# SpectacularAI/HybVIO

Measured on AMD Instinct MI355X. Metric: VIO frames/sec at 752x480 stereo, 200 KLT features; pyramid+KLT HBM GB/s, higher is better.
Workload: dtype u8/int16 pixels, int32/int64 sums, f32 solve (tracker); f64 (EKF); 1 GPU; C3: 752x480 stereo, 200 pts -- the whole frame chained on one stream per sequence: 2 pyramid builds, temporal LK from predicted positions, 2-point rotation RANSAC on its output, stereo LK, GFTT key points every 2nd frame (HIP tracker), then the HIP EKF from the device mean: 20 track visits (triangulation + prepareVisualUpdate + chi2 gate; track lengths 5 + Geometric(0.2) <= 21 stereo poses = 20 .~; sequences_per_gpu=4096, engines_per_gpu=4, parallelism=replicas x1 (no collective)

## Files before the change

### hybvio_amd/csrc/ekf.hip

```cpp
#include <functional>
#include <limits.h>
#include <math.h>

#include <utility>

#include <stdlib.h>

#include "ekf_device.hpp"

#pragma clang fp contract(fast)

namespace hv {

namespace {


}
__device__ long long g_phase_stamp[16];
namespace {
#ifdef HV_EKF_PHASE_STAMPS
#define PHASE_STAMP(i) do { if (blockIdx.x == 0 && threadIdx.x == 0) g_phase_stamp[i] = (long long)__builtin_readcyclecounter(); } while (0)
#else
#define PHASE_STAMP(i) do { } while (0)
#endif
// ... 496 lines not shown
        }
        __syncthreads();
        for (int w = t; w < ns * 12; w += 256) {
            const int sl = w / 12, tt = w - 12 * sl;
            double *const sh = shs + sl * SHW;
            if (sh[X_LIVE] == 0.0) continue;
            double *const F = Fs + sl * INER * INER;
            const double *const sA = sh, *const sT34 = sh + 88;
            const int i = tt / 4, j = tt - 4 * i;
            double s_ = 0; for (int k = 0; k < 4; k++) s_ += sT34[3 * k + i] * sA[4 * j + k];
            F_(VEL + i, ORI + j) = s_;
        }
        __syncthreads();
        for (int w = t; w < ns * 32; w += 256) {
            const int sl = w >> 5, tt = w & 31;
            double *const sh = shs + sl * SHW;
            if (sh[X_LIVE] == 0.0) continue;
            double *const F = Fs + sl * INER * INER, *const Lm = Ls + sl * INER * QD;
            if (tt < 9) {
                const int i = tt / 3, g = tt - 3 * i;
                double s_ = 0; for (int k = 0; k < 4; k++) s_ += F_(VEL + i, ORI + k) * L_(ORI + k, Q_GYRO + g);
                L_(VEL + i, Q_GYRO + g) = s_;
                F_(VEL + i, BGA + g) = -s_;
            } else if (tt >= 16 && tt < 28) {
                const int e = tt - 16, i = e / 3, g = e - 3 * i;
                F_(ORI + i, BGA + g) = -L_(ORI + i, Q_GYRO + g);
            }
        }
        if (s0 == 0) PHASE_STAMP(6);
        int last_live = -1;
        bool q_set = false;
        auto set_q = [&](const double *sh_q) {
            if (a.baa > 0.0 && t < 9) { const int i = t % 3, j = t / 3; Qs[(Q_BAA_DRIFT + j) * QD + Q_BAA_DRIFT + i] = (i == j) ? sh_q[X_VBAA] : 0.0; }
            if (a.bga > 0.0 && t >= 16 && t < 25) { const int e = t - 16, i = e % 3, j = e / 3; Qs[(Q_BGA_DRIFT + j) * QD + Q_BGA_DRIFT + i] = (i == j) ? sh_q[X_VBGA] : 0.0; }
        };
        for (int sl = 0; sl < ns; sl++) {
            double *const sh = shs + sl * SHW;
            __syncthreads();
            if (sh[X_LIVE] == 0.0) continue;
            last_live = sl;
            const double *const F = Fs + sl * INER * INER, *const Lm = Ls + sl * INER * QD;
            if (!q_set) { set_q(sh); __syncthreads(); }
            q_set = false;
            if (s0 == 0 && sl == 1) PHASE_STAMP(7);
            const int ti = wave & 1, tj = wave >> 1;
            const int mi = ti ? INER - 16 : 16, nj = tj ? INER - 16 : 16;
            const double4v fp = mfma_tile<5>(F + 16 * ti, 1, INER, mi, P00 + 16 * tj * INER, 1, INER, nj, INER);
            const double4v ph = mfma_tile<5>(F + 16 * ti, 1, INER, mi, Phi + 16 * tj * INER, 1, INER, nj, INER);
            double4v lq = {0.0, 0.0, 0.0, 0.0};
            if (wave < 2) lq = mfma_tile<3>(Lm + 16 * wave, 1, INER, wave ? INER - 16 : 16, Qs, 1, QD, QD, QD);
#pragma unroll
            for (int q = 0; q < 4; q++) {
                const int r = kq + 4 * q;
                if (r < mi && cl < nj) { FP[(16 * tj + cl) * INER + 16 * ti + r] = fp[q]; PhiN[(16 * tj + cl) * INER + 16 * ti + r] = ph[q]; }
                if (wave < 2 && r < (wave ? INER - 16 : 16) && cl < QD) LQ[cl * INER + 16 * wave + r] = lq[q];
            }
            if (s0 == 0 && sl == 1) PHASE_STAMP(8);
            __syncthreads();
            if (s0 == 0 && sl == 1) PHASE_STAMP(9);
            {
                int nx = sl + 1;
                while (nx < ns && shs[nx * SHW + X_LIVE] == 0.0) nx++;
                if (nx < ns) { set_q(shs + nx * SHW); q_set = true; }
            }
            const double4v p1 = mfma_tile<5>(FP + 16 * ti, 1, INER, mi, F + 16 * tj, INER, 1, nj, INER);
            const double4v p2 = mfma_tile<3>(LQ + 16 * ti, 1, INER, mi, Lm + 16 * tj, INER, 1, nj, QD);
#pragma unroll
            for (int q = 0; q < 4; q++) {
                const int r = kq + 4 * q;
                if (r < mi && cl < nj) P00[(16 * tj + cl) * INER + 16 * ti + r] = p1[q] + p2[q];
            }
            for (int e = t; e < INER * INER; e += 256) Phi[e] = PhiN[e];
            if (s0 == 0 && sl == 1) PHASE_STAMP(10);
        }
        __syncthreads();
        if (s0 == 0) PHASE_STAMP(11);
        if (last_live >= 0)
            for (int i = t; i < INER * INER; i += 256) a.dydx[(size_t)b * INER * INER + i] = Fs[last_live * INER * INER + i];
        __syncthreads();
    }
    for (int i = t; i < INER * INER; i += 256) P[(size_t)(i / INER) * n + (i % INER)] = P00[i];
    for (int i = t; i < QD * QD; i += 256) Q[i] = Qs[i];
    if (t < INER) m[t] = ms[t];
    PHASE_STAMP(14);
    {
        double f0[5], f1[5];
#pragma unroll
        for (int sx = 0; sx < 5; sx++) {
            const int k = 4 * sx + kq;
            f0[sx] = Phi[k * INER + cl];
            f1[sx] = Phi[k * INER + min(16 + cl, INER - 1)];
        }
        for (int base = 0; base < 2 * tiles; base += 4 * NIT) {
#pragma unroll
            for (int u = 0; u < NIT; u++) {
                const int it = base + wave + 4 * u;
                if (it < 2 * tiles) {
                    if (base > 0) {
#pragma unroll
                        for (int sx = 0; sx < 5; sx++) slab[u][sx] = *slab_ptr(it, sx);
                    }
                    double4v a0 = {0.0, 0.0, 0.0, 0.0}, a1 = a0;
                    const bool p10 = it < tiles;
#pragma unroll
                    for (int sx = 0; sx < 5; sx++) {
                        const double x0 = p10 ? f0[sx] : slab[u][sx], y0 = p10 ? slab[u][sx] : f0[sx];
                        const double x1 = p10 ? f1[sx] : slab[u][sx], y1 = p10 ? slab[u][sx] : f1[sx];
                        a0 = __builtin_amdgcn_mfma_f64_16x16x4f64(x0, y0, a0, 0, 0, 0);
                        a1 = __builtin_amdgcn_mfma_f64_16x16x4f64(x1, y1, a1, 0, 0, 0);
                    }
#pragma unroll
                    for (int q = 0; q < 4; q++) {
                        const int rr = kq + 4 * q;
                        if (p10) {
                            const int i = INER + 16 * it + cl;
                            if (i < n) {
                                P[(size_t)rr * n + i] = a0[q];
                                if (16 + rr < INER) P[(size_t)(16 + rr) * n + i] = a1[q];
                            }
                        } else {
                            const int c = INER + 16 * (it - tiles) + rr;
                            if (c < n) {
                                P[(size_t)c * n + cl] = a0[q];
                                if (16 + cl < INER) P[(size_t)c * n + 16 + cl] = a1[q];
                            }
                        }
                    }
                }
            }
        }
    }
    __syncthreads();
    PHASE_STAMP(15);
}

struct UpdateArgs {
    int n, nr, l, R, Rs;
    int mode;
    int generic;
    int normalize_all, use_lds, map_dim;
    double *m, *P;
    const double *H, *v;
    const double *rdiag;
    double rd0, noise_scale;
    double rd1;
    double *ws;
    double *chi2; int *status;
    const unsigned char *active;
    const int *require_inlier;
    int *success_counter;
    int spec, n_tracks, max_successful;
    int *cursor;
    const int *gate_in;
    const int *nr_rec;
    int *cursor_out;
    int *pub;
    int pass_id;
    int *err;
    const int *acol;
    int na_max, ncam;
    size_t h_stride;
    int v_stride;
    int half, nr_full;
    double *dm_out; const double *dm_in;
    int *gate_rw;
    int half_auto; int *sel_io;
    int *epoch;
    int batch;
    const int *rec_count, *rec_list;
};

__device__ __forceinline__ void spec_publish(const UpdateArgs &a, int rec, int code)
{
    __hip_atomic_store(a.pub + rec, a.pass_id * 4 + code, __ATOMIC_RELEASE, __HIP_MEMORY_SCOPE_AGENT);
}
__device__ __forceinline__ int spec_wait(const UpdateArgs &a, int rec)
{
    for (int spin = 0; spin < (1 << 20); ++spin) {
        const int v = __hip_atomic_load(a.pub + rec, __ATOMIC_ACQUIRE, __HIP_MEMORY_SCOPE_AGENT);
        if ((v >> 2) == a.pass_id) return v & 3;
        __builtin_amdgcn_s_sleep(8);
    }
    if (a.err) atomicOr(a.err, 1);
    return -1;
}
__device__ __forceinline__ void spec_close(const UpdateArgs &a, int b, int c0, bool pass_ran)
{
    bool any = false;
    for (int jj = c0; jj < a.n_tracks - 1 && !any; ++jj) any = spec_wait(a, jj * (int)gridDim.x + b) == 2;
    if (!any) a.cursor_out[b] = pass_ran ? a.n_tracks : c0;
}

constexpr int UPD_THREADS = 512;

template <int MODE, int TI, bool AUTO = false>
__device__ __forceinline__ void ekf_update_body(const UpdateArgs &a, const int b_in )
{
    const int b = __builtin_amdgcn_readfirstlane(b_in);
    constexpr bool USE_LDS = MODE >= 1;
    extern __shared__ __attribute__((aligned(16))) double smem[];
    int e = b;
    int sel = -1;
    if (a.spec == 1) {
        const int j = blockIdx.y;
        if (j < a.cursor[b] || a.success_counter[b] >= a.max_successful) return;
        e = j * (int)gridDim.x + b;
    } else if (AUTO && a.spec == 2 && a.half == 2) {
        sel = a.sel_io[b];
        if (sel < 0) return;
        e = sel * (int)gridDim.x + b;
        if (a.gate_in[e] != 0) {
            if (threadIdx.x == 0) a.cursor[b] = sel + 1;
            return;
        }
    } else if (a.spec == 2) {
        const int c0 = a.cursor[b];
        if (AUTO && threadIdx.x == 0) a.sel_io[b] = -1;
        if (c0 >= a.n_tracks || a.success_counter[b] >= a.max_successful) return;
        for (int j = c0; j < a.n_tracks && sel < 0; ++j) {
            const int ee = j * (int)gridDim.x + b;
            if (a.active[ee] && a.gate_in[ee] == 0) sel = j;
        }
        if (sel < 0) {
            __syncthreads();
            if (threadIdx.x == 0) a.cursor[b] = a.n_tracks;
            return;
        }
        e = sel * (int)gridDim.x + b;
    }
    int c0_spec = 0;
    if (a.spec == 3) {
        const int j = blockIdx.y;
        c0_spec = a.cursor[b];
        e = j * (int)gridDim.x + b;
        const bool pass_runs = c0_spec < a.n_tracks && a.success_counter[b] < a.max_successful;
        if (!pass_runs || j < c0_spec || !a.active[e]) {
            if (threadIdx.x == 0) {
                spec_publish(a, e, 1);
                if (j == a.n_tracks - 1) spec_close(a, b, c0_spec, pass_runs);
            }
            return;
        }
    }
    const int t = threadIdx.x, lane = t & 63;
    const unsigned char act_v = a.active ? a.active[e] : (unsigned char)1;
    const int req_v = a.require_inlier ? a.require_inlier[b] : 0;
    const int nr_rec_v0 = a.nr_rec ? a.nr_rec[e] : a.nr_full;
    int shape_pin = nr_rec_v0;
    asm volatile("" : "+v"(shape_pin));
    const int nr_rec_v = shape_pin;
    if (!act_v) return;
    if (req_v != 0) return;
#ifdef HV_DEBUG_SKIP_UPDATE
    if (a.mode == 1 && a.spec == 0) { if (a.success_counter && t == 0) a.success_counter[b] += 1; return; }
#endif
    const int wave = __builtin_amdgcn_readfirstlane(t >> 6);
    constexpr int nwaves = UPD_THREADS / 64;
    const int n = a.n, l = a.l;
    int nr = a.nr, R = a.Rs, Rfull = a.R;
    int roff = 0, ld = a.nr;
    int half = a.half;
    if (a.nr_rec || a.half) {
        int nr_full = __builtin_amdgcn_readfirstlane(nr_rec_v);
        if (nr_full < 1 || nr_full > a.v_stride) return;
        nr = nr_full; ld = nr_full;
        if constexpr (AUTO) {
            if (nr_full <= 48) {
                if (half == 2) return;
                half = 0;
            }
            if (half == 1 && t == 0) a.sel_io[b] = sel;
        }
        if (half) {
            if (MODE != 2) return;
            const int h1 = 2 * ((nr_full + 3) >> 2);
            roff = half == 2 ? h1 : 0;
            nr = half == 2 ? nr_full - h1 : h1;
        }
        if (nr < 1 || nr > a.nr) return;
        Rfull = nr + n + 1; R = Rfull;
        if (USE_LDS) while ((R & 31) != 15 && (R & 31) != 17) R++;
    }
    double *m = a.m + (size_t)b * n, *P = a.P + (size_t)b * n * n;
    const double *H = a.H + (size_t)e * a.h_stride;
    const double rd = a.rdiag ? a.rdiag[b] : a.rd0;
    double *T = USE_LDS ? smem : a.ws + (size_t)b * a.Rs * a.nr;
    double *W = USE_LDS ? smem + (((size_t)R * nr + 1) & ~(size_t)1) : smem;
    double *col = W + 256;
    double *red = col + 544;
    int *s_stop = reinterpret_cast<int *>(red + nwaves);
    double *Hs = red + nwaves + 2;
    constexpr int nrp = 16 * (TI > 0 ? TI : 1);
    const bool gate_only = a.mode == 0;
    const int rv = nr, ry = nr + 1;
    const bool two_r = MODE == 2 && a.mode == 3;
    int Rlim = (gate_only || two_r) ? nr + 1 : Rfull;

    PHASE_STAMP(0);
    const int kq = lane >> 4, cl = lane & 15;
    constexpr int NBK = 10, NBH = 5;
    double pres0[NBK][4], pres1[NBH][4];
    const int tiles_j = (n + 15) >> 4, lb = (l + 15) >> 4;
    const int hs = (tiles_j + 1) >> 1;
    const int J1 = 8 + (wave & 1), kb0_1 = (wave & 2) ? hs : 0, kb1_1 = (wave & 2) ? tiles_j : hs;
    const bool have0 = MODE == 2 && wave < tiles_j, have1 = MODE == 2 && wave < 4 && J1 < tiles_j;
    unsigned kbmask = 0xFFFFFFFFu;
    if constexpr (MODE == 2) {
        auto fetch_blk = [&](auto &pv, int bi, int J, int kb, int kend) {
            if (kb < kend && (kb < lb || !gate_only)) {
                const int jc = min(J * 16 + cl, n - 1);
#pragma unroll
                for (int sx = 0; sx < 4; sx++)
                    pv[bi][sx] = *reinterpret_cast<const double *>(reinterpret_cast<const char *>(P) + (unsigned)(min(kb * 16 + 4 * sx + kq, n - 1) * n + jc) * 8u);
            }
        };
        constexpr int HREG = (48 * 160 + UPD_THREADS - 1) / UPD_THREADS, DEPTH = 4;
        if (a.acol) {
            int *mask = reinterpret_cast<int *>(col);
            const int na = 7 * (ld / (2 * a.ncam)) + 1;
            const int *acol = a.acol + (size_t)e * a.na_max;
            const int total = na * nr;
            const unsigned inv_nr = (unsigned)((0x100000000ull + (unsigned)nr - 1) / (unsigned)nr);
            constexpr int HC = 8;
            double hv[HC]; int hc[HC];
            auto request = [&](int base) {
#pragma unroll
                for (int u = 0; u < HC; u++) {
                    const int i = base + t + u * UPD_THREADS, uc = (int)__umulhi((unsigned)i, inv_nr), r = i - uc * nr;
                    const bool live = i < total;
                    hc[u] = live ? acol[uc] : -1;
                    hv[u] = live ? *reinterpret_cast<const double *>(reinterpret_cast<const char *>(H) + (unsigned)(uc * ld + roff + r) * 8u) : 0.0;
                }
            };
            auto scatter = [&](int base) {
#pragma unroll
                for (int u = 0; u < HC; u++) {
                    const int i = base + t + u * UPD_THREADS, uc = (int)__umulhi((unsigned)i, inv_nr), r = i - uc * nr;
                    if (hc[u] >= 0 && hc[u] < l) {
                        Hs[hc[u] * nrp + r] = hv[u];
                        if (r == 0) atomicOr(mask, 1 << (hc[u] >> 4));
                    }
                }
            };
            request(0);
#pragma unroll
            for (int bi = DEPTH - 1; bi >= 0; bi--) if (have0) fetch_blk(pres0, bi, wave, bi, tiles_j);
            PHASE_STAMP(8);
            for (int i = t; i < nrp * 16 * lb; i += UPD_THREADS) Hs[i] = 0.0;
            for (int i = t; i < R * nr; i += UPD_THREADS) T[i] = 0.0;
            if (t == 0) mask[0] = 0;
            __syncthreads();
            scatter(0);
            for (int base = HC * UPD_THREADS; base < total; base += HC * UPD_THREADS) { request(base); scatter(base); }
            __syncthreads();
            kbmask = (unsigned)mask[0];
        } else {
            double hreg[HREG];
#pragma unroll
            for (int u = 0; u < HREG; u++) {
                const int i = t + u * UPD_THREADS, k = i / nrp, r = i - k * nrp;
                hreg[u] = (i < nrp * 16 * lb && k < l && r < nr) ? H[(size_t)k * ld + roff + r] : 0.0;
            }
#pragma unroll
            for (int bi = 0; bi < DEPTH; bi++) if (have0) fetch_blk(pres0, bi, wave, bi, tiles_j);
            PHASE_STAMP(8);
            for (int i = t; i < R * nr; i += UPD_THREADS) T[i] = 0.0;
#pragma unroll
            for (int u = 0; u < HREG; u++) {
                const int i = t + u * UPD_THREADS;
                if (i < nrp * 16 * lb) Hs[i] = hreg[u];
            }
        }
        __syncthreads();
        PHASE_STAMP(9);
        const double *hbase = Hs + (size_t)kq * nrp + cl;
        auto load_h = [&](int kb, int hf, double (&av)[2][TI]) {
#pragma unroll
            for (int sx = 0; sx < 2; sx++)
#pragma unroll
                for (int mt = 0; mt < TI; mt++) av[sx][mt] = hbase[(size_t)(kb * 16 + 4 * (2 * hf + sx)) * nrp + 16 * mt];
        };
        auto mfma_half = [&](auto &pv, int bi, int hf, const double (&av)[2][TI], double4v (&acc)[TI]) {
#pragma unroll
            for (int sx = 0; sx < 2; sx++)
#pragma unroll
                for (int mt = 0; mt < TI; mt++)
                    acc[mt] = __builtin_amdgcn_mfma_f64_16x16x4f64(av[sx][mt], pv[bi][2 * hf + sx], acc[mt], 0, 0, 0);
        };
        auto flush = [&](int J, double4v (&acc)[TI]) {
#pragma unroll
            for (int mt = 0; mt < TI; mt++) {
#pragma unroll
                for (int q = 0; q < 4; q++) {
                    const int i = 16 * mt + kq + 4 * q, j = J * 16 + cl;
                    if (i < nr && j < n) unsafeAtomicAdd(&T[(size_t)i * R + ry + j], acc[mt][q]);
                }
            }
        };
        {
            double4v acc[TI];
#pragma unroll
            for (int mt = 0; mt < TI; mt++) acc[mt] = double4v{0.0, 0.0, 0.0, 0.0};
            const int nv = have0 ? min(tiles_j, lb) : 0;
            double av[2][2][TI];
            if (nv > 0) load_h(0, 0, av[0]);
#pragma unroll
            for (int bi = 0; bi < NBK; bi++) {
                if (bi + DEPTH < NBK) { if (have0) fetch_blk(pres0, bi + DEPTH, wave, bi + DEPTH, tiles_j); }
                else if (bi + DEPTH - NBK < NBH) { if (have1) fetch_blk(pres1, bi + DEPTH - NBK, J1, kb0_1 + bi + DEPTH - NBK, kb1_1); }
                if (bi < nv) {
                    const bool work = (kbmask >> bi) & 1;
                    load_h(bi, 1, av[1]);
                    if (work) mfma_half(pres0, bi, 0, av[0], acc);
                    if (bi + 1 < nv) load_h(bi + 1, 0, av[0]);
                    if (work) mfma_half(pres0, bi, 1, av[1], acc);
                }
            }
            if (have0) flush(wave, acc);
        }
        PHASE_STAMP(10);
        {
            double4v acc[TI];
#pragma unroll
            for (int mt = 0; mt < TI; mt++) acc[mt] = double4v{0.0, 0.0, 0.0, 0.0};
            const int nv = have1 ? max(min(kb1_1, lb) - kb0_1, 0) : 0;
            double av[2][2][TI];
            if (nv > 0) load_h(kb0_1, 0, av[0]);
#pragma unroll
            for (int bi = 0; bi < NBH; bi++) {
                if (bi + DEPTH < NBH) { if (have1) fetch_blk(pres1, bi + DEPTH, J1, kb0_1 + bi + DEPTH, kb1_1); }
                if (bi < nv) {
                    const bool work = (kbmask >> (kb0_1 + bi)) & 1;
                    load_h(kb0_1 + bi, 1, av[1]);
                    if (work) mfma_half(pres1, bi, 0, av[0], acc);
                    if (bi + 1 < nv) load_h(kb0_1 + bi + 1, 0, av[0]);
                    if (work) mfma_half(pres1, bi, 1, av[1], acc);
                }
            }
            if (have1) flush(J1, acc);
        }
        PHASE_STAMP(11);
    } else {
        const int tiles_i = (nr + 15) / 16;
        for (int tile = wave; tile < tiles_i * tiles_j; tile += nwaves) {
            const int i0 = (tile % tiles_i) * 16, j0 = (tile / tiles_i) * 16;
            const double4v acc = mfma_tile<8>(H + i0, 1, nr, nr - i0, P + j0, n, 1, n - j0, l);
            const int j = j0 + cl;
#pragma unroll
            for (int q = 0; q < 4; q++) {
                const int i = i0 + kq + 4 * q;
                if (i < nr && j < n) T[(size_t)i * R + ry + j] = acc[q];
            }
        }
    }
    for (int i = t; i < nr; i += UPD_THREADS) {
        double r = a.v[(size_t)e * a.v_stride + roff + i];
        if (a.generic) { double s = 0; for (int k = 0; k < l; k++) s += H[(size_t)k * nr + i] * m[k]; r -= s; }
        if constexpr (MODE == 2) {
            if (a.dm_in) {
                const double *dm = a.dm_in + (size_t)b * n;
                double s = 0;
                for (int k = 0; k < l; k++) s += Hs[(size_t)k * nrp + i] * dm[k];
                r -= s;
            }
        }
        T[(size_t)i * R + rv] = r;
    }
    __syncthreads();

    PHASE_STAMP(1);
    {
        const int tb = (nr + 15) / 16;
        if constexpr (MODE == 2) {
            const int khalf = ((l / 2) + 15) & ~15;
            for (int it = wave; it < tb * (tb + 1); it += nwaves) {
                const int hh = it & 1;
                int ib = it >> 1, cb = 0;
                while (ib >= tb - cb) { ib -= tb - cb; cb++; }
                ib += cb;
                const int i0 = ib * 16, c0 = cb * 16;
                const int kbeg = hh ? min(khalf, l) : 0, klen = hh ? l - kbeg : min(khalf, l);
                if (klen <= 0) continue;
                const double *pa = T + (size_t)min(i0 + cl, nr - 1) * R + ry + kbeg + kq;
                const double *pb = Hs + (size_t)(kbeg + kq) * nrp + c0 + cl;
                double4v acc = {0.0, 0.0, 0.0, 0.0};
                for (int k0 = 0; k0 < klen; k0 += 32) {
                    double av[8], bv[8];
#pragma unroll
                    for (int u = 0; u < 8; u++) {
                        const bool live = k0 + 4 * u < klen;
                        const int kk = live ? k0 + 4 * u : 0;
                        av[u] = pa[kk]; bv[u] = pb[(size_t)kk * nrp];
                        if (!live) bv[u] = 0.0;
                    }
#pragma unroll
                    for (int u = 0; u < 8; u++) acc = __builtin_amdgcn_mfma_f64_16x16x4f64(av[u], bv[u], acc, 0, 0, 0);
                }
                const int c = c0 + cl;
#pragma unroll
                for (int q = 0; q < 4; q++) {
                    const int i = i0 + kq + 4 * q;
                    if (i < nr && c < nr) unsafeAtomicAdd(&T[(size_t)c * R + i], acc[q] + ((i == c && hh == 0) ? rd : 0.0));
                }
            }
        } else {
            for (int tile = wave; tile < tb * tb; tile += nwaves) {
                const int ib = tile % tb, cb = tile / tb;
                if (ib < cb) continue;
                const int i0 = ib * 16, c0 = cb * 16;
                const double4v acc = mfma_tile<8>(T + (size_t)i0 * R + ry, R, 1, nr - i0, H + c0, nr, 1, nr - c0, l);
                const int c = c0 + cl;
#pragma unroll
                for (int q = 0; q < 4; q++) {
                    const int i = i0 + kq + 4 * q;
                    if (i < nr && c < nr) T[(size_t)c * R + i] = acc[q] + (i == c ? rd : 0.0);
                }
            }
        }
    }
    __syncthreads();
    if constexpr (MODE == 2) {
        if (two_r) {
            for (int e = t; e < (nr + 1) * nr; e += UPD_THREADS) { const int c = e / (nr + 1), i = e - c * (nr + 1); Hs[256 + e] = T[(size_t)c * R + i]; }
            __syncthreads();
        }
    }

    PHASE_STAMP(2);
    for (int pass = 0; pass < (two_r ? 2 : 1); ++pass) {
    for (int j0 = 0; j0 < nr; j0 += 16) {
        const int w = min(16, nr - j0);
        const int ntile = (Rlim - j0 + 15) / 16;
        const int i_l = lane >> 4, c_l = lane & 15;
        if (j0 > 0) {
            for (int tile = wave; tile < ntile; tile += nwaves) {
                const int i0 = j0 + 16 * tile, mi = Rlim - i0;
                const double4v acc = mfma_tile(T + i0, 1, R, mi, T + j0, R, 1, w, j0);
#pragma unroll
                for (int q = 0; q < 4; q++) {
                    const int i = i_l + 4 * q;
                    if (i < mi && c_l < w) T[(size_t)(j0 + c_l) * R + i0 + i] -= acc[q];
                }
            }
            __syncthreads();
        }
        if (j0 == 0) PHASE_STAMP(6);
        if (wave == 0) { if (w <= 8) factor_diag_block<8>(T, W, col, R, j0, w, lane); else factor_diag_block<16>(T, W, col, R, j0, w, lane); }
        __syncthreads();
        if (j0 == 0) PHASE_STAMP(7);
        for (int i0 = j0 + w + 16 * wave; i0 < Rlim; i0 += 16 * nwaves) {
            const int mi = Rlim - i0;
            const double4v acc = mfma_tile(T + (size_t)j0 * R + i0, 1, R, mi, W, 16, 1, 16, w);
#pragma unroll
            for (int q = 0; q < 4; q++) {
                const int i = i_l + 4 * q;
                if (i < mi && c_l < w) T[(size_t)(j0 + c_l) * R + i0 + i] = acc[q];
            }
        }
        __syncthreads();
    }

    PHASE_STAMP(3);
    {
        double s = 0;
        for (int c = t; c < nr; c += UPD_THREADS) { const double z = T[(size_t)c * R + rv]; s += z * z; }
        for (int o = 32; o > 0; o >>= 1) s += __shfl_down(s, o);
        if (lane == 0) red[wave] = s;
        __syncthreads();
        if (t == 0) {
            double tot = 0; for (int w2 = 0; w2 < nwaves; w2++) tot += red[w2];
            tot *= a.noise_scale;
            const bool broken = !(tot < 1e300);
            const int outlier = broken || ((nr < HV_CHI2INV95_N) ? (tot > d_chi2inv95[nr]) : 0);
            if (pass == 0) {
                if (a.chi2) a.chi2[e] = tot;
                if (a.status) a.status[e] = outlier ? 3  : 0 ;
            }
            *s_stop = (a.mode == 0) || broken || ((a.mode == 2 || (two_r && pass == 0)) && outlier);
            if (broken && a.gate_rw) a.gate_rw[e] = 3 ;
            if (AUTO && broken && a.spec == 2 && half != 1) a.cursor[b] = sel + 1;
            if (AUTO && broken && a.spec == 2 && half == 2 && a.epoch)
                for (int jj = sel + 1; jj < a.n_tracks; ++jj) a.epoch[jj * (int)gridDim.x + b] = -1;
            if (a.spec == 3 && pass == 0) {
                const int j = blockIdx.y;
                spec_publish(a, e, outlier ? 1 : 2);
                if (!outlier) {
                    bool lose = false;
                    for (int jj = c0_spec; jj < j && !lose; ++jj) lose = spec_wait(a, jj * (int)gridDim.x + b) != 1;
                    if (lose) *s_stop = 1;
                }
                if (*s_stop && j == a.n_tracks - 1 && outlier) spec_close(a, b, c0_spec, true);
            }
            if (a.spec == 3 && pass == 1 && *s_stop) a.cursor_out[b] = (int)blockIdx.y + 1;
        }
        __syncthreads();
        if (*s_stop) return;
    }
    if constexpr (MODE == 2) {
        if (two_r && pass == 0) {
            const double shift = a.rd1 - rd;
            for (int e = t; e < (nr + 1) * nr; e += UPD_THREADS) {
                const int c = e / (nr + 1), i = e - c * (nr + 1);
                T[(size_t)c * R + i] = Hs[256 + e] + (i == c ? shift : 0.0);
            }
            Rlim = Rfull;
            __syncthreads();
        }
    }
    }

    PHASE_STAMP(4);
    for (int j = t; j < n; j += UPD_THREADS) {
        double s = 0;
        for (int c = 0; c < nr; c++) s += T[(size_t)c * R + ry + j] * T[(size_t)c * R + rv];
        m[j] += s;
        if (a.dm_out && !(AUTO && half == 0)) a.dm_out[(size_t)b * n + j] = s;
    }
    if constexpr (MODE == 2) {
        auto down_item = [&](auto &pv, int nblk, int J, int kb0, int kb1) {
            const int jc = min(J * 16 + cl, n - 1);
            constexpr int KS = 4 * TI;
            double yj[KS];
#pragma unroll
            for (int sx = 0; sx < KS; sx++) {
                const int c = 4 * sx + kq;
                const double y = T[(size_t)min(c, nr - 1) * R + ry + jc];
                yj[sx] = c < nr ? y : 0.0;
            }
#pragma unroll
            for (int bi = 0; bi < nblk; bi++) {
                const int kb = kb0 + bi;
                if (kb < kb1) {
                    const int ic = min(kb * 16 + cl, n - 1);
                    double av[KS];
#pragma unroll
                    for (int sx = 0; sx < KS; sx++) av[sx] = T[(size_t)min(4 * sx + kq, nr - 1) * R + ry + ic];
                    double4v acc = {0.0, 0.0, 0.0, 0.0};
#pragma unroll
                    for (int sx = 0; sx < KS; sx++) {
                        if (sx < KS - 4 || 4 * sx < nr) acc = __builtin_amdgcn_mfma_f64_16x16x4f64(av[sx], yj[sx], acc, 0, 0, 0);
                    }
#pragma unroll
                    for (int q = 0; q < 4; q++) {
                        const int i = kb * 16 + kq + 4 * q, j = J * 16 + cl;
                        if (i < n && j < n) P[(size_t)i * n + j] = pv[bi][q] - acc[q];
                    }
                }
            }
        };
        if (have0) down_item(pres0, NBK, wave, 0, tiles_j);
        if (have1) down_item(pres1, NBH, J1, kb0_1, kb1_1);
    } else {
        const int tb = (n + 15) / 16, ntiles = tb * tb;
        const int cj = lane & 15, ri = lane >> 4;
        auto p_addr = [&](int tile, int q) -> double * {
            const int i = min((tile % tb) * 16 + ri + 4 * q, n - 1), j = min((tile / tb) * 16 + cj, n - 1);
            return P + (size_t)i * n + j;
        };
        double cur[4], nxt[4] = {0.0, 0.0, 0.0, 0.0};
        if (wave < ntiles) {
#pragma unroll
            for (int q = 0; q < 4; q++) cur[q] = *p_addr(wave, q);
        }
        for (int tile = wave; tile < ntiles; tile += nwaves) {
            const int i0 = (tile % tb) * 16, j0 = (tile / tb) * 16;
            const int tn = min(tile + nwaves, ntiles - 1);
#pragma unroll
            for (int q = 0; q < 4; q++) nxt[q] = *p_addr(tn, q);
            const double4v acc = mfma_tile(T + ry + i0, 1, R, n - i0, T + ry + j0, R, 1, n - j0, nr);
#pragma unroll
            for (int q = 0; q < 4; q++) {
                const int i = i0 + ri + 4 * q, j = j0 + cj;
                if (i < n && j < n) P[(size_t)i * n + j] = cur[q] - acc[q];
                cur[q] = nxt[q];
            }
        }
    }
    __syncthreads();
    PHASE_STAMP(5);
    const bool first_block = AUTO ? half == 1 : a.normalize_all < 0;
    const int nq = first_block ? 0 : (a.normalize_all != 0) ? 1 + (n - a.map_dim - CAM) / POSE : 1;
    if (t < nq) normalize4(m + (t == 0 ? ORI : CAM + POSE * (t - 1) + 3));
    if (a.success_counter && t == 0 && !(AUTO && half == 1)) a.success_counter[b] += 1;
    if (a.spec == 2 && t == 0 && !(AUTO && half == 1)) a.cursor[b] = sel + 1;
    if (a.spec == 3 && t == 0) a.cursor_out[b] = (int)blockIdx.y + 1;
}

template <int MODE, int TI>
__global__ __launch_bounds__(UPD_THREADS) void ekf_update_kernel(UpdateArgs a)
{
    int b = blockIdx.x;
    if (a.rec_list) { if ((int)blockIdx.x >= *a.rec_count) return; b = a.rec_list[blockIdx.x]; }
    ekf_update_body<MODE, TI>(a, b);
}

__global__ __launch_bounds__(UPD_THREADS) void ekf_update_spec_long_kernel(UpdateArgs a)
{
    ekf_update_body<2, 3, true>(a, blockIdx.x);
}

struct UpdatePair { UpdateArgs a[2]; };
template <int MODE, int TI>
__global__ __launch_bounds__(UPD_THREADS) void ekf_update_dual_kernel(UpdatePair p, int part, int num_cus)
{
    const int n0 = *p.a[0].rec_count, n1 = *p.a[1].rec_count, i = (int)blockIdx.x;
    const int cap = min(n0, max(num_cus - n1, 0));
    const int lo = part == 1 ? cap : 0, hi = part == 0 ? cap : n0;
    const bool second = i < n1;
    const UpdateArgs &a = p.a[second ? 1 : 0];
    const int j = second ? i : i - n1 + lo;
    if (!second && j >= hi) return;
    ekf_update_body<MODE, TI>(a, a.rec_list[j]);
}


struct GateArgs {
    int n, nr, l, Rs;
    const double *P;
    const double *H, *v;
    double rd, noise_scale;
    double *chi2; int *status;
    const unsigned char *active;
    const int *success_counter; int max_successful;
};

constexpr int GATE_THREADS = 256;

template <int TI>
__global__ __launch_bounds__(GATE_THREADS, 2) void ekf_gate_stream_kernel(GateArgs a)
{
    extern __shared__ __attribute__((aligned(16))) double smem[];
    const int b = blockIdx.x;
    if (a.active && !a.active[b]) return;
    if (a.success_counter && a.success_counter[b] >= a.max_successful) return;
    const int t = threadIdx.x, lane = t & 63;
    const int wave = __builtin_amdgcn_readfirstlane(t >> 6);
    constexpr int nwaves = GATE_THREADS / 64, nrp = 16 * TI;
    const int n = a.n, nr = a.nr, l = a.l, R = a.Rs;
    const double *P = a.P + (size_t)b * n * n, *H = a.H + (size_t)b * nr * l;
    const int lb = (l + 15) >> 4;
    double *Hs = smem, *T = smem + (size_t)nrp * 16 * lb;
    const int kq = lane >> 4, cl = lane & 15;
    for (int i = t; i < nrp * 16 * lb; i += GATE_THREADS) {
        const int k = i / nrp, r = i - k * nrp;
        Hs[i] = (k < l && r < nr) ? H[(size_t)k * nr + r] : 0.0;
    }
    for (int i = t; i < R * nr; i += GATE_THREADS) T[i] = 0.0;
    __syncthreads();
    double4v accS[TI * (TI + 1) / 2];
#pragma unroll
    for (int u = 0; u < TI * (TI + 1) / 2; u++) accS[u] = double4v{0.0, 0.0, 0.0, 0.0};
    constexpr int DEPTH = 4;
    for (int J = wave; J < lb; J += nwaves) {
        const int jrow = min(J * 16 + cl, n - 1);
        auto fetch = [&](double (&pv)[4], int kb) {
#pragma unroll
            for (int sx = 0; sx < 4; sx++) pv[sx] = P[(size_t)min(kb * 16 + 4 * sx + kq, n - 1) * n + jrow];
        };
        double pv[DEPTH][4];
#pragma unroll
        for (int d = 0; d < DEPTH; d++) if (d < lb) fetch(pv[d], d);
        double4v accG[TI];
#pragma unroll
        for (int ct = 0; ct < TI; ct++) accG[ct] = double4v{0.0, 0.0, 0.0, 0.0};
        for (int kb0 = 0; kb0 < lb; kb0 += DEPTH) {
#pragma unroll
            for (int d = 0; d < DEPTH; d++) {
                const int kb = kb0 + d;
                if (kb < lb) {
                    double hb[4][TI];
#pragma unroll
                    for (int sx = 0; sx < 4; sx++)
#pragma unroll
                        for (int ct = 0; ct < TI; ct++) hb[sx][ct] = Hs[(size_t)(kb * 16 + 4 * sx + kq) * nrp + 16 * ct + cl];
#pragma unroll
                    for (int sx = 0; sx < 4; sx++)
#pragma unroll
                        for (int ct = 0; ct < TI; ct++)
                            accG[ct] = __builtin_amdgcn_mfma_f64_16x16x4f64(pv[d][sx], hb[sx][ct], accG[ct], 0, 0, 0);
                    if (kb + DEPTH < lb) fetch(pv[d], kb + DEPTH);
                }
            }
        }
        if (J * 16 < n) {
#pragma unroll
            for (int v = 0; v < 4; v++) {
                double ha[TI];
#pragma unroll
                for (int rt = 0; rt < TI; rt++) ha[rt] = Hs[(size_t)(J * 16 + 4 * v + kq) * nrp + 16 * rt + cl];
                int u = 0;
#pragma unroll
                for (int ct = 0; ct < TI; ct++)
#pragma unroll
                    for (int rt = ct; rt < TI; rt++, u++)
                        accS[u] = __builtin_amdgcn_mfma_f64_16x16x4f64(ha[rt], accG[ct][v], accS[u], 0, 0, 0);
            }
        }
    }
    for (int w_turn = 0; w_turn < nwaves; ++w_turn) {
        if (wave == w_turn) {
            int u = 0;
#pragma unroll
            for (int ct = 0; ct < TI; ct++)
#pragma unroll
                for (int rt = ct; rt < TI; rt++, u++)
#pragma unroll
                    for (int q = 0; q < 4; q++) {
                        const int i = 16 * rt + kq + 4 * q, c = 16 * ct + cl;
                        if (i < nr && c < nr && i >= c) T[(size_t)c * R + i] += accS[u][q];
                    }
        }
        __syncthreads();
    }
    for (int i = t; i < nr; i += GATE_THREADS) { T[(size_t)i * R + i] += a.rd; T[(size_t)i * R + nr] = a.v[(size_t)b * nr + i]; }
    double *W = Hs, *col = Hs + 256, *red = Hs + 256 + 544;
    __syncthreads();
    const int Rlim = nr + 1;
    for (int j0 = 0; j0 < nr; j0 += 16) {
        const int w = min(16, nr - j0);
        const int ntile = (Rlim - j0 + 15) / 16;
        if (j0 > 0) {
            for (int tile = wave; tile < ntile; tile += nwaves) {
                const int i0 = j0 + 16 * tile, mi = Rlim - i0;
                const double4v acc = mfma_tile(T + i0, 1, R, mi, T + j0, R, 1, w, j0);
#pragma unroll
                for (int q = 0; q < 4; q++) {
                    const int i = kq + 4 * q;
                    if (i < mi && cl < w) T[(size_t)(j0 + cl) * R + i0 + i] -= acc[q];
                }
            }
            __syncthreads();
        }
        if (wave == 0) { if (w <= 8) factor_diag_block<8>(T, W, col, R, j0, w, lane); else factor_diag_block<16>(T, W, col, R, j0, w, lane); }
        __syncthreads();
        for (int i0 = j0 + w + 16 * wave; i0 < Rlim; i0 += 16 * nwaves) {
            const int mi = Rlim - i0;
            const double4v acc = mfma_tile(T + (size_t)j0 * R + i0, 1, R, mi, W, 16, 1, 16, w);
#pragma unroll
            for (int q = 0; q < 4; q++) {
                const int i = kq + 4 * q;
                if (i < mi && cl < w) T[(size_t)(j0 + cl) * R + i0 + i] = acc[q];
            }
        }
        __syncthreads();
    }
    double sz = 0;
    for (int c = t; c < nr; c += GATE_THREADS) { const double z = T[(size_t)c * R + nr]; sz += z * z; }
    for (int o = 32; o > 0; o >>= 1) sz += __shfl_down(sz, o);
    if (lane == 0) red[wave] = sz;
    __syncthreads();
    if (t == 0) {
        double tot = 0; for (int w2 = 0; w2 < nwaves; w2++) tot += red[w2];
        tot *= a.noise_scale;
        if (a.chi2) a.chi2[b] = tot;
        if (a.status) a.status[b] = tot > d_chi2inv95[nr] ? 3  : 0 ;
    }
}

struct SparseGateArgs {
    int n, nr, ncam, na_max;
    const double *P;
    const double *Hc, *v;
    const int *acol;
    const int *nr_rec;
    const unsigned char *active;
    double rd, noise_scale;
    double *chi2; int *status;
    int hs_doubles;
    int lds_doubles;
    int batch;
    const int *rec_count, *rec_list;
    int *inl_count, *inl_list;
};

constexpr int SGATE_THREADS = 256;
constexpr int SGATE_BIG_THREADS = 768;

template <bool BIG>
__device__ __forceinline__ void sparse_gate_kernel_body(const SparseGateArgs &a, const int b_in)
{
    const int b = __builtin_amdgcn_readfirstlane(b_in);
    extern __shared__ __attribute__((aligned(16))) double smem[];
    const int t = threadIdx.x;
    constexpr int NTH = BIG ? SGATE_BIG_THREADS : SGATE_THREADS;
    PHASE_STAMP(12);
    const unsigned char act_v = a.active[b];
    const int nr_v = a.nr_rec ? a.nr_rec[b] : a.nr;
    int my_acol_raw = a.acol[(size_t)b * a.na_max + min(t, a.na_max - 1)];
    double my_v_raw = a.v[(size_t)b * a.nr + min(t, a.nr - 1)];
    asm volatile("" : "+v"(my_acol_raw), "+v"(my_v_raw));
    if (!act_v) return;
    const int nr = __builtin_amdgcn_readfirstlane(nr_v);
    if (nr < 2 || nr > a.nr) return;
    const int n = a.n, npose = nr / (2 * a.ncam), na = 7 * npose + 1, na4 = (na + 3) & ~3;
    const int ti = BIG ? max((nr + 15) >> 4, 4) : (nr + 15) >> 4;
    int Rs = nr + 1;
    while ((Rs & 31) != 15 && (Rs & 31) != 17) Rs++;
    const bool tight = BIG && (size_t)na4 * 16 * ti + (size_t)Rs * nr > (size_t)a.lds_doubles;
    if (tight) Rs = nr + 1 + ((nr + 1) & 1 ? 0 : 1);
    if (tight && nr > HV_GATE_TIGHT_ROWS) return;
    const int nrp = tight ? HV_GATE_TIGHT_ROWS : 16 * ti;
    double *Hs = smem, *T = smem + a.hs_doubles;
    int *s_acol = reinterpret_cast<int *>(T + (size_t)Rs * nr);
    const double *Hc = a.Hc + (size_t)b * a.nr * a.na_max;
    const int my_acol = t < na ? my_acol_raw : 0;
    const double my_v = t < nr ? my_v_raw : 0.0;
    const int total = na4 * nrp;
    const unsigned inv_nrp = (unsigned)((0x100000000ull + (unsigned)nrp - 1) / (unsigned)nrp);
    for (int base = 0; base < total; base += 8 * NTH) {
        double hv_[8];
#pragma unroll
        for (int q = 0; q < 8; q++) {
            const int i = base + q * NTH + t, u = (int)__umulhi((unsigned)i, inv_nrp), r = i - u * nrp;
            const bool live = i < total && u < na && r < nr;
            hv_[q] = live ? Hc[(size_t)(live ? u : 0) * nr + (live ? r : 0)] : 0.0;
        }
#pragma unroll
        for (int q = 0; q < 8; q++) {
            const int i = base + q * NTH + t;
            if (i < total) Hs[i] = hv_[q];
        }
    }
    for (int i = t; i < Rs * nr; i += NTH) T[i] = 0.0;
    if (t < na) s_acol[t] = my_acol;
    __syncthreads();
    if (t < nr) T[(size_t)t * Rs + nr] = my_v;
    __syncthreads();
    PHASE_STAMP(13);
    const double *Pb = a.P + (size_t)b * n * n;
    double chi;
    if constexpr (!BIG) {
        if (ti == 1)      chi = sparse_gate<1, NTH, true>(Pb, n, s_acol, na, Hs, T, Rs, nr, a.rd, a.noise_scale, Hs, BIG ? g_phase_stamp : nullptr);
        else if (ti == 2) chi = sparse_gate<2, NTH, true>(Pb, n, s_acol, na, Hs, T, Rs, nr, a.rd, a.noise_scale, Hs, BIG ? g_phase_stamp : nullptr);
        else              chi = sparse_gate<3, NTH, true>(Pb, n, s_acol, na, Hs, T, Rs, nr, a.rd, a.noise_scale, Hs, BIG ? g_phase_stamp : nullptr);
    } else {
        if (ti <= 4)      chi = sparse_gate<4, NTH, false>(Pb, n, s_acol, na, Hs, T, Rs, nr, a.rd, a.noise_scale, Hs, BIG ? g_phase_stamp : nullptr);
        else if (ti == 5) chi = sparse_gate<5, NTH, false>(Pb, n, s_acol, na, Hs, T, Rs, nr, a.rd, a.noise_scale, Hs, BIG ? g_phase_stamp : nullptr);
        else if (!tight)  chi = sparse_gate<6, NTH, false>(Pb, n, s_acol, na, Hs, T, Rs, nr, a.rd, a.noise_scale, Hs, BIG ? g_phase_stamp : nullptr);
        else              chi = sparse_gate<6, NTH, false, true>(Pb, n, s_acol, na, Hs, T, Rs, nr, a.rd, a.noise_scale, Hs, BIG ? g_phase_stamp : nullptr);
    }
    if (t == 0) {
        const bool broken = !(chi < 1e300);
        const int outlier = broken || ((nr < HV_CHI2INV95_N) ? (chi > d_chi2inv95[nr]) : 0);
        a.status[b] = outlier ? 3  : 0 ;
        if (!outlier && a.inl_list) a.inl_list[atomicAdd(a.inl_count, 1)] = b;
        if (a.chi2) a.chi2[b] = chi;
    }
}

__global__ __launch_bounds__(SGATE_THREADS, 3) void ekf_sparse_gate_kernel(SparseGateArgs a) { sparse_gate_kernel_body<false>(a, blockIdx.x); }
__global__ __launch_bounds__(SGATE_BIG_THREADS, 1) void ekf_sparse_gate_big_kernel(SparseGateArgs a)
{
    int b = blockIdx.x;
    if (a.rec_list) { if (b >= *a.rec_count) return; b = a.rec_list[b]; }
// ... 1818 lines not shown
```

Baseline: 152,300 frames/s.

## Exploit covariance symmetry in EKF P downdate and skip unneeded P tile fetches

The covariance downdate now computes only lower-triangular tiles (kb >= J) and mirrors each value into the upper triangle, so roughly half the MFMA downdate work is skipped. Column tiles are reassigned across waves (J0 = wave or 11-wave) to balance the triangular workload, and the second-half item starts late. P block prefetches for off-triangle blocks are now skipped unless the H sparsity mask needs them for the T = H·P product. In exchange, every thread writes both P[i][j] and P[j][i], which is scattered transposed traffic. Correctness depends on P being exactly symmetric, and on the kbmask value being valid at the time of the prefetch.

Result: faster. 154,000 frames/s, median of 6 (+1.1%).

```diff
diff --git a/hybvio_amd/csrc/ekf.hip b/hybvio_amd/csrc/ekf.hip
--- a/hybvio_amd/csrc/ekf.hip
+++ b/hybvio_amd/csrc/ekf.hip
@@ -822,12 +822,14 @@
     double pres0[NBK][4], pres1[NBH][4];
     const int tiles_j = (n + 15) >> 4, lb = (l + 15) >> 4;
     const int hs = (tiles_j + 1) >> 1;
+    const int J0 = wave < 4 ? wave : 11 - wave;
     const int J1 = 8 + (wave & 1), kb0_1 = (wave & 2) ? hs : 0, kb1_1 = (wave & 2) ? tiles_j : hs;
-    const bool have0 = MODE == 2 && wave < tiles_j, have1 = MODE == 2 && wave < 4 && J1 < tiles_j;
+    const bool have0 = MODE == 2 && J0 < tiles_j, have1 = MODE == 2 && wave < 4 && J1 < tiles_j;
     unsigned kbmask = 0xFFFFFFFFu;
     if constexpr (MODE == 2) {
         auto fetch_blk = [&](auto &pv, int bi, int J, int kb, int kend) {
-            if (kb < kend && (kb < lb || !gate_only)) {
+            const bool hp = kb < lb && ((kbmask >> kb) & 1);
+            if (kb < kend && (kb >= J ? (hp || !gate_only) : hp)) {
                 const int jc = min(J * 16 + cl, n - 1);
 #pragma unroll
                 for (int sx = 0; sx < 4; sx++)
@@ -864,7 +866,7 @@
             };
             request(0);
 #pragma unroll
-            for (int bi = DEPTH - 1; bi >= 0; bi--) if (have0) fetch_blk(pres0, bi, wave, bi, tiles_j);
+            for (int bi = DEPTH - 1; bi >= 0; bi--) if (have0) fetch_blk(pres0, bi, J0, bi, tiles_j);
             PHASE_STAMP(8);
             for (int i = t; i < nrp * 16 * lb; i += UPD_THREADS) Hs[i] = 0.0;
             for (int i = t; i < R * nr; i += UPD_THREADS) T[i] = 0.0;
@@ -882,7 +884,7 @@
                 hreg[u] = (i < nrp * 16 * lb && k < l && r < nr) ? H[(size_t)k * ld + roff + r] : 0.0;
             }
 #pragma unroll
-            for (int bi = 0; bi < DEPTH; bi++) if (have0) fetch_blk(pres0, bi, wave, bi, tiles_j);
+            for (int bi = 0; bi < DEPTH; bi++) if (have0) fetch_blk(pres0, bi, J0, bi, tiles_j);
             PHASE_STAMP(8);
             for (int i = t; i < R * nr; i += UPD_THREADS) T[i] = 0.0;
 #pragma unroll
@@ -926,7 +928,7 @@
             if (nv > 0) load_h(0, 0, av[0]);
 #pragma unroll
             for (int bi = 0; bi < NBK; bi++) {
-                if (bi + DEPTH < NBK) { if (have0) fetch_blk(pres0, bi + DEPTH, wave, bi + DEPTH, tiles_j); }
+                if (bi + DEPTH < NBK) { if (have0) fetch_blk(pres0, bi + DEPTH, J0, bi + DEPTH, tiles_j); }
                 else if (bi + DEPTH - NBK < NBH) { if (have1) fetch_blk(pres1, bi + DEPTH - NBK, J1, kb0_1 + bi + DEPTH - NBK, kb1_1); }
                 if (bi < nv) {
                     const bool work = (kbmask >> bi) & 1;
@@ -936,7 +938,7 @@
                     if (work) mfma_half(pres0, bi, 1, av[1], acc);
                 }
             }
-            if (have0) flush(wave, acc);
+            if (have0) flush(J0, acc);
         }
         PHASE_STAMP(10);
         {
@@ -1137,7 +1139,7 @@
         if (a.dm_out && !(AUTO && half == 0)) a.dm_out[(size_t)b * n + j] = s;
     }
     if constexpr (MODE == 2) {
-        auto down_item = [&](auto &pv, int nblk, int J, int kb0, int kb1) {
+        auto down_item = [&](auto &pv, int nblk, int b0, int J, int kb0, int kb1) {
             const int jc = min(J * 16 + cl, n - 1);
             constexpr int KS = 4 * TI;
             double yj[KS];
@@ -1148,9 +1150,9 @@
                 yj[sx] = c < nr ? y : 0.0;
             }
 #pragma unroll
-            for (int bi = 0; bi < nblk; bi++) {
+            for (int bi = b0; bi < nblk; bi++) {
                 const int kb = kb0 + bi;
-                if (kb < kb1) {
+                if (kb >= J && kb < kb1) {
                     const int ic = min(kb * 16 + cl, n - 1);
                     double av[KS];
 #pragma unroll
@@ -1163,13 +1165,17 @@
 #pragma unroll
                     for (int q = 0; q < 4; q++) {
                         const int i = kb * 16 + kq + 4 * q, j = J * 16 + cl;
-                        if (i < n && j < n) P[(size_t)i * n + j] = pv[bi][q] - acc[q];
+                        const double v = pv[bi][q] - acc[q];
+                        if (i < n && j < n && i >= j) {
+                            P[(size_t)i * n + j] = v;
+                            if (i > j) P[(size_t)j * n + i] = v;
+                        }
                     }
                 }
             }
         };
-        if (have0) down_item(pres0, NBK, wave, 0, tiles_j);
-        if (have1) down_item(pres1, NBH, J1, kb0_1, kb1_1);
+        if (have0) down_item(pres0, NBK, 0, J0, 0, tiles_j);
+        if (have1) down_item(pres1, NBH, NBH - 2, J1, kb0_1, kb1_1);
     } else {
         const int tb = (n + 15) / 16, ntiles = tb * tb;
         const int cj = lane & 15, ri = lane >> 4;
```
